# RishWijewardhena/vision-textile-inspection

Measured on AMD Instinct MI355X. Metric: frames/sec whole-node, YOLOv8n-seg 640x640 bs=64; mask IoU vs CPU ref, higher is better.
Workload: dtype f16x2

## Files before the change

include/vti.h:

```cpp
#ifndef VTI_H
#define VTI_H

#include <stddef.h>
#include <stdint.h>

#ifdef __cplusplus
extern "C" {
#endif

typedef struct vti_ctx vti_ctx;

typedef enum {
    VTI_OK = 0,
    VTI_ERR_ARG = -1,
    VTI_ERR_STATE = -2,
    VTI_ERR_WEIGHTS = -3,
    VTI_ERR_HIP = -4,
    VTI_ERR_NOMEM = -5,
    VTI_ERR_UNSUPPORTED = -6
} vti_status;

enum { VTI_F16 = 0, VTI_F32 = 1, VTI_H2 = 2 };
enum { VTI_MASK_LOGIT = 0,
       VTI_MASK_SIGMOID = 1 };
// ... 323 lines not shown
    const int32_t* classes;
} vti_nms_params;
VTI_NMS_TABLE_API int64_t vti_nms_table_bytes(int32_t n_rows);
VTI_NMS_TABLE_API int32_t vti_pack_nms_table(vti_ctx* ctx, const vti_nms_params* params, int32_t n_rows,
                                             void* host_table, size_t nbytes);
VTI_NMS_TABLE_API int32_t vti_set_nms_table(vti_ctx* ctx, const void* host_table, const void* dev_table,
                                            int32_t n_rows, const int32_t* dev_row_of_frame);

#define VTI_WINDOWS_API
VTI_WINDOWS_API int64_t vti_window_table_bytes(int32_t B);
VTI_WINDOWS_API int32_t vti_pack_windows(vti_ctx* ctx, int32_t H, int32_t W, const int32_t* H0, const int32_t* W0,
                                         const int64_t* byte_offset, const int32_t* windows, int32_t B, int64_t total_bytes,
                                         void* host_table, size_t nbytes);
VTI_WINDOWS_API int32_t vti_window_table_info(const void* host_table, int32_t b, int32_t out_i32[12], double out_f64[5]);
VTI_WINDOWS_API int32_t vti_letterbox_windows(vti_ctx* ctx, const uint8_t* dev_frames, const void* host_table, const void* dev_table,
                                              int32_t B, uint8_t* dev_input, void* stream);
VTI_WINDOWS_API int32_t vti_scale_boxes_windows(vti_ctx* ctx, const float* dev_dets, const int32_t* dev_counts, const void* host_table,
                                                const void* dev_table, int32_t B, int32_t max_det, float* dev_xyxy, void* stream);
VTI_WINDOWS_API int64_t vti_mask_native_windows_bytes(const vti_ctx* ctx, const void* host_table, int32_t max_det);
VTI_WINDOWS_API int32_t vti_masks_native_windows(vti_ctx* ctx, const float* dev_dets, const int32_t* dev_counts, const void* dev_proto,
                                                 const void* host_table, const void* dev_table, int32_t B, int32_t max_det, int32_t mode,
                                                 int32_t packing, uint8_t* dev_masks, int64_t capacity_bytes, int32_t* dev_offsets,
                                                 int64_t* dev_mask_bases, void* stream);
VTI_WINDOWS_API int32_t vti_predict_windows(vti_ctx* ctx, const uint8_t* dev_frames, const void* host_table, const void* dev_table,
                                            int32_t B, int32_t swap_rb, float conf, double iou, int32_t max_det, int32_t agnostic,
                                            int32_t mask_mode, int32_t packing, uint8_t* dev_input_scratch, float* dev_pred,
                                            void* dev_proto, float* dev_dets, int32_t* dev_counts, uint8_t* dev_masks,
                                            int64_t capacity_bytes, int32_t* dev_offsets, int64_t* dev_mask_bases, float* dev_xyxy,
                                            void* stream);

#define VTI_ANNOTATE_NATIVE_API
VTI_ANNOTATE_NATIVE_API int32_t vti_annotate_frames_native(vti_ctx* ctx, const uint8_t* dev_frames, const void* host_table,
                                                           const void* dev_table, int32_t B, const void* dev_cameras, int32_t n_cams,
                                                           const int32_t* dev_camera_of_frame, const uint8_t* dev_masks,
                                                           const int64_t* dev_mask_bases, int64_t capacity_bytes, const float* dev_dets,
                                                           const float* dev_xyxy, const int32_t* dev_counts, const int32_t* dev_offsets,
                                                           int32_t max_det, int32_t capacity, const int32_t* frame_i32,
                                                           const double* stitch_f64, const int32_t* stitch_i32,
                                                           const int32_t* host_select, const int32_t* dev_select, int32_t n_sel,
                                                           int32_t max_points, const void* host_out_table, const void* dev_out_table,
                                                           uint8_t* dev_out, int32_t* dev_status, void* dev_scratch, size_t scratch_bytes,
                                                           void* stream);
VTI_ANNOTATE_NATIVE_API int32_t vti_annotate_checker_frames_native(vti_ctx* ctx, const uint8_t* dev_frames, const void* host_table,
                                                                   const void* dev_table, int32_t B, const void* dev_cameras,
                                                                   int32_t n_cams, const int32_t* dev_camera_of_frame,
                                                                   const uint8_t* dev_masks, const int64_t* dev_mask_bases,
                                                                   int64_t capacity_bytes, const float* dev_dets, const float* dev_xyxy,
                                                                   const int32_t* dev_counts, const int32_t* dev_offsets, int32_t max_det,
                                                                   int32_t capacity, const int32_t* frame_i32, const double* stitch_f64,
                                                                   const int32_t* stitch_i32, const int32_t* host_select,
                                                                   const int32_t* dev_select, int32_t n_sel, int32_t max_points,
                                                                   const void* host_out_table, const void* dev_out_table,
                                                                   uint8_t* dev_out, int32_t* dev_status, void* dev_scratch,
                                                                   size_t scratch_bytes, void* stream);

int64_t vti_decode_jpeg_table_bytes(int32_t n);
int32_t vti_decode_jpeg_plan(vti_ctx* ctx, const uint8_t* host_files, const int64_t* host_file_offsets, int32_t n,
                             int32_t segment_bytes, int32_t layout, void* host_table, size_t nbytes, int32_t* out_H0,
                             int32_t* out_W0, int64_t* out_byte_offsets, int64_t* out_scratch_bytes);
enum { VTI_JPEG_CORRUPT = 1 };
int32_t vti_decode_jpeg(vti_ctx* ctx, const uint8_t* dev_files, const void* host_table, const void* dev_table, int32_t n, int32_t rgb,
                        uint8_t* dev_out, int64_t out_bytes, int32_t* dev_info, void* dev_scratch, size_t scratch_bytes, void* stream);

enum { VTI_RAW_YUYV = 0, VTI_RAW_UYVY, VTI_RAW_NV12, VTI_RAW_NV21, VTI_RAW_I420, VTI_RAW_YV12 };
int64_t vti_raw_frame_bytes(int32_t fmt, int32_t H0, int32_t W0);
int32_t vti_convert_raw(vti_ctx* ctx, const uint8_t* dev_raw, int32_t fmt, int32_t B, int32_t H0, int32_t W0, int32_t rgb,
                        uint8_t* dev_frames, void* stream);
int64_t vti_raw_table_bytes(int32_t n);
int32_t vti_pack_raw_frames(vti_ctx* ctx, const int32_t* H0, const int32_t* W0, const int32_t* fmt, int32_t n, void* host_raw_table,
                            size_t nbytes, int64_t* out_raw_offsets);
int32_t vti_convert_raw_frames(vti_ctx* ctx, const uint8_t* dev_raw, int64_t raw_bytes, const void* host_raw_table,
                               const void* dev_raw_table, const void* host_frame_table, const void* dev_frame_table, int32_t n,
                               int32_t rgb, uint8_t* dev_out, int64_t out_bytes, void* stream);

int32_t vti_debug_conv_output(vti_ctx* ctx, int32_t i, int32_t B, float* dev_out, void* stream);

int32_t vti_debug_conv2d(int32_t dtype, const void* dev_in, int32_t B, int32_t H, int32_t W, int32_t in_ld,
                         int32_t in_coff, int32_t c1, const float* host_w, const float* host_b, int32_t c2,
                         int32_t k, int32_t s, int32_t kind, const void* dev_res, int32_t res_ld, int32_t res_coff,
                         void* dev_out, int32_t out_ld, int32_t out_coff, int32_t out_f32, int32_t swap_rb,
                         int32_t tile_h, int32_t tile_w, int32_t waves_n, int32_t nrep, int32_t iters,
                         float* ms_out, int32_t* cfg_out, void* stream);

#ifdef __cplusplus
}
#endif
#endif
```

vision-textile-inspection_amd/_lib.py:

```python
import ctypes as C
import os

_HERE = os.path.dirname(os.path.abspath(__file__))
_VARIANT = os.environ.get("VTI_LIB_VARIANT", "")
LIB_PATH = os.path.join(_HERE, f"libvti_{_VARIANT}.so" if _VARIANT else "libvti.so")

VTI_F16, VTI_F32, VTI_H2 = 0, 1, 2
VTI_MASK_LOGIT, VTI_MASK_SIGMOID = 0, 1
VTI_PACK_U8, VTI_PACK_BITS = 0, 1
VTI_MASK_NATIVE = 0x10


class VtiDesc(C.Structure):
    _fields_ = [("scale", C.c_char), ("nc", C.c_int32), ("nm", C.c_int32), ("reg_max", C.c_int32),
                ("H", C.c_int32), ("W", C.c_int32), ("max_batch", C.c_int32), ("dtype", C.c_int32)]


class VtiConvInfo(C.Structure):
    _fields_ = [("name", C.c_char * 48), ("c1", C.c_int32), ("c2", C.c_int32), ("k", C.c_int32),
                ("s", C.c_int32), ("kind", C.c_int32), ("h_in", C.c_int32), ("w_in", C.c_int32),
                ("h_out", C.c_int32), ("w_out", C.c_int32), ("macs", C.c_int64),
                ("tile_h", C.c_int32), ("tile_w", C.c_int32), ("waves_n", C.c_int32), ("nrep", C.c_int32),
                ("lds_bytes", C.c_int32), ("fused", C.c_int32), ("persistent", C.c_int32)]

# ... 90 lines not shown
                                   _P, _P, _P, _P, _P]),
    "vti_frame_table_bytes": (_I64, [_I32]),
    "vti_pack_frames": (_I32, [_P, _I32, _I32, _P, _P, _P, _I32, _I64, _P, _SZ]),
    "vti_frame_table_info": (_I32, [_P, _I32, _P, _P]),
    "vti_letterbox_frames": (_I32, [_P, _P, _P, _P, _I32, _P, _P]),
    "vti_scale_boxes_frames": (_I32, [_P, _P, _P, _P, _P, _I32, _I32, _P, _P]),
    "vti_predict_frames": (_I32, [_P, _P, _P, _P, _I32, _I32, _F, _D, _I32, _I32, _I32, _I32,
                                  _P, _P, _P, _P, _P, _P, _I32, _P, _P, _P]),
    "vti_measure_frames": (_I32, [_P, _P, _I32, _P, _P, _I32, _P, _P, _P, _P, _P, _P, _I32, _I32, _I32, _P, _SZ,
                                  _P, _P, _P, _P, _P]),
    "vti_mask_native_frames_bytes": (_I64, [_P, _P, _I32]),
    "vti_masks_native_frames": (_I32, [_P, _P, _P, _P, _P, _P, _P, _I32, _I32, _I32, _I32, _P, _I64, _P, _P, _P]),
    "vti_predict_frames_native": (_I32, [_P, _P, _P, _P, _I32, _I32, _F, _D, _I32, _I32, _I32, _I32,
                                         _P, _P, _P, _P, _P, _P, _I64, _P, _P, _P, _P]),
    "vti_measure_frames_native": (_I32, [_P, _P, _I32, _P, _P, _P, _I64, _P, _P, _P, _P, _P, _P, _I32, _I32, _I32, _P, _SZ,
                                         _P, _P, _P, _P, _P]),
    "vti_mask_polygons_scratch_bytes": (_I64, [_P, _I32, _I32, _I32]),
    "vti_mask_polygons": (_I32, [_P, _P, _I32, _P, _I32, _I32, _I32, _I32, _I32, _I32, _P, _SZ, _P, _P, _I64, _P]),
    "vti_mask_polygons_frames_scratch_bytes": (_I64, [_P, _P, _I32]),
    "vti_mask_polygons_frames": (_I32, [_P, _P, _I32, _P, _I64, _P, _P, _P, _I32, _I32, _I32, _P, _SZ, _P, _P, _I64, _P]),
    "vti_annotate_scratch_bytes": (_I64, [_P, _I32, _I32, _I32, _I32, _I32]),
    "vti_annotate": (_I32, [_P, _P, _I32, _I32, _I32, _P, _I32, _P, _P, _I32, _P, _P, _P, _P, _I32, _I32, _P, _P, _P, _P, _P, _I32,
                            _I32, _P, _P, _P, _SZ, _P]),
    "vti_annotate_frames_scratch_bytes": (_I64, [_P, _P, _I32, _I32]),
    "vti_annotate_frames": (_I32, [_P, _P, _P, _P, _I32, _P, _I32, _P, _P, _I32, _P, _P, _P, _P, _I32, _I32, _P, _P, _P, _P, _P, _I32,
                                   _I32, _P, _P, _P, _P, _P, _SZ, _P]),
    "vti_annotate_checker": (_I32, [_P, _P, _I32, _I32, _I32, C.POINTER(VtiCheckerParams), _P, _I32, _P, _P, _P, _P, _I32, _I32, _P, _P, _P,
                                    _P, _P, _I32, _I32, _P, _P, _P, _SZ, _P]),
    "vti_checker_pack_cameras": (_I32, [_P, C.POINTER(VtiCheckerParams), _I32, _P, _SZ]),
    "vti_measure_checker_cameras": (_I32, [_P, _P, _I32, _P, _P, _I32, _P, _P, _P, _P, _I32, _I32, _I32, _I32, _I32, _P, _SZ,
                                           _P, _P, _P, _P, _P]),
    "vti_measure_checker_frames": (_I32, [_P, _P, _I32, _P, _P, _I32, _P, _P, _P, _P, _P, _P, _I32, _I32, _I32, _P, _SZ,
                                          _P, _P, _P, _P, _P]),
    "vti_measure_checker_frames_native": (_I32, [_P, _P, _I32, _P, _P, _P, _I64, _P, _P, _P, _P, _P, _P, _I32, _I32, _I32, _P, _SZ,
                                                 _P, _P, _P, _P, _P]),
    "vti_annotate_checker_cameras": (_I32, [_P, _P, _I32, _I32, _I32, _P, _I32, _P, _P, _I32, _P, _P, _P, _P, _I32, _I32, _P, _P, _P,
                                            _P, _P, _I32, _I32, _P, _P, _P, _SZ, _P]),
    "vti_annotate_checker_frames": (_I32, [_P, _P, _P, _P, _I32, _P, _I32, _P, _P, _I32, _P, _P, _P, _P, _I32, _I32, _P, _P, _P, _P, _P,
                                           _I32, _I32, _P, _P, _P, _P, _P, _SZ, _P]),
    "vti_annotate_frames_native": (_I32, [_P, _P, _P, _P, _I32, _P, _I32, _P, _P, _P, _I64, _P, _P, _P, _P, _I32, _I32, _P, _P, _P, _P, _P,
                                          _I32, _I32, _P, _P, _P, _P, _P, _SZ, _P]),
    "vti_annotate_checker_frames_native": (_I32, [_P, _P, _P, _P, _I32, _P, _I32, _P, _P, _P, _I64, _P, _P, _P, _P, _I32, _I32, _P, _P, _P,
                                                  _P, _P, _I32, _I32, _P, _P, _P, _P, _P, _SZ, _P]),
    "vti_overlay_scratch_bytes": (_I64, [_P, _I32, _I32, _I32, _I32, _I32]),
    "vti_overlay": (_I32, [_P, _P, _I32, _I32, _I32, _P, _I32, _P, _P, _P, _P, _I32, _I32, _P, _P, _I32, _F, _F, _P, _P, _I32, _I32, _P,
                           _I32, _P, _P, _P, _SZ, _P]),
    "vti_overlay_frames_scratch_bytes": (_I64, [_P, _P, _I32, _I32]),
    "vti_overlay_frames": (_I32, [_P, _P, _P, _P, _I32, _P, _I32, _P, _I64, _P, _P, _P, _P, _I32, _I32, _P, _P, _I32, _F, _F, _P, _P, _I32,
                                  _I32, _P, _I32, _P, _P, _P, _P, _P, _SZ, _P]),
    "vti_encode_jpeg_scratch_bytes": (_I64, [_P, _I32, _I32, _I32]),
    "vti_encode_jpeg_max_bytes": (_I64, [_I32, _I32, _I32]),
    "vti_encode_jpeg": (_I32, [_P, _P, _I32, _I32, _I32, _I32, _I32, _P, _SZ, _P, _P, _I64, _P]),
    "vti_encode_jpeg_frames_scratch_bytes": (_I64, [_P, _P]),
    "vti_encode_jpeg_frames_max_bytes": (_I64, [_P]),
    "vti_encode_jpeg_frames": (_I32, [_P, _P, _P, _P, _I32, _I32, _I32, _P, _SZ, _P, _P, _I64, _P]),
    "vti_stamp_table_bytes": (_I64, [_I32, _I32]),
    "vti_pack_stamps": (_I32, [_P, _P, _P, _I32, _P, _I32, _I64, _P, _SZ]),
    "vti_stamp": (_I32, [_P, _P, _I32, _I32, _I32, _P, _P, _P, _I64, _P]),
    "vti_stamp_frames": (_I32, [_P, _P, _P, _P, _I32, _P, _P, _P, _I64, _P]),
    "vti_nms_table_bytes": (_I64, [_I32]),
    "vti_pack_nms_table": (_I32, [_P, C.POINTER(VtiNmsParams), _I32, _P, _SZ]),
    "vti_set_nms_table": (_I32, [_P, _P, _P, _I32, _P]),
    "vti_window_table_bytes": (_I64, [_I32]),
    "vti_pack_windows": (_I32, [_P, _I32, _I32, _P, _P, _P, _P, _I32, _I64, _P, _SZ]),
    "vti_window_table_info": (_I32, [_P, _I32, _P, _P]),
    "vti_letterbox_windows": (_I32, [_P, _P, _P, _P, _I32, _P, _P]),
    "vti_scale_boxes_windows": (_I32, [_P, _P, _P, _P, _P, _I32, _I32, _P, _P]),
    "vti_mask_native_windows_bytes": (_I64, [_P, _P, _I32]),
    "vti_masks_native_windows": (_I32, [_P, _P, _P, _P, _P, _P, _I32, _I32, _I32, _I32, _P, _I64, _P, _P, _P]),
    "vti_predict_windows": (_I32, [_P, _P, _P, _P, _I32, _I32, _F, _D, _I32, _I32, _I32, _I32,
                                   _P, _P, _P, _P, _P, _P, _I64, _P, _P, _P, _P]),
    "vti_decode_jpeg_table_bytes": (_I64, [_I32]),
    "vti_decode_jpeg_plan": (_I32, [_P, _P, _P, _I32, _I32, _I32, _P, _SZ, _P, _P, _P, _P]),
    "vti_decode_jpeg": (_I32, [_P, _P, _P, _P, _I32, _I32, _P, _I64, _P, _P, _SZ, _P]),
    "vti_raw_frame_bytes": (_I64, [_I32, _I32, _I32]),
    "vti_convert_raw": (_I32, [_P, _P, _I32, _I32, _I32, _I32, _I32, _P, _P]),
    "vti_raw_table_bytes": (_I64, [_I32]),
    "vti_pack_raw_frames": (_I32, [_P, _P, _P, _P, _I32, _P, _SZ, _P]),
    "vti_convert_raw_frames": (_I32, [_P, _P, _I64, _P, _P, _P, _P, _I32, _I32, _P, _I64, _P]),
    "vti_debug_conv_output": (_I32, [_P, _I32, _I32, _P, _P]),
    "vti_debug_conv2d": (_I32, [_I32, _P, _I32, _I32, _I32, _I32, _I32, _I32, _P, _P, _I32, _I32, _I32, _I32,
                                _P, _I32, _I32, _P, _I32, _I32, _I32, _I32, _I32, _I32, _I32, _I32, _I32,
                                _P, _P, _P]),
}

_lib = None


def lib():
    global _lib
    if _lib is None:
        if not os.path.exists(LIB_PATH):
            raise ImportError(f"{LIB_PATH} not found: build it with `python -c 'import __graft_entry__ as g; "
                              f"g.build()'` (hipcc --offload-arch=gfx950); there is no CPU fallback")
        L = C.CDLL(LIB_PATH)
        for name, (res, args) in SIGNATURES.items():
            fn = getattr(L, name)
            fn.restype, fn.argtypes = res, args
        _lib = L
    return _lib


def check(ctx, rc):
    if rc != 0:
        msg = lib().vti_last_error(ctx)
        raise VtiError(rc, msg.decode() if msg else "")
```

vision-textile-inspection_amd/api.py:

```python
from ._lib import LIB_PATH, SIGNATURES, VtiError, lib
from .engine import Engine, FrameTable, WindowTable, NmsParams, NmsTable, RawTable, StampTable, debug_conv2d, h2_decode, h2_encode, kmeans1d2, pixels_to_world, unpack_bits
from .feeder import FrameFeeder
from .model import YOLO, Boxes, Masks, RawFrames, Results, letterbox_shape
from .weights import pack_container, random_weights, unpack_container
from .convert import convert_checkpoint, convert_state_dict
from .measure import CheckerParams, MeasureParams, MultiCameraChecker, MultiCameraMeasurer, StitchDistanceChecker, StitchMeasurer, checker_text_items
from .annotate import checker_display_list
from . import annotate, consumer, dataparallel, jpeg, overlay, rawframes

__all__ = ["LIB_PATH", "SIGNATURES", "VtiError", "lib", "Engine", "FrameTable", "WindowTable", "NmsParams", "NmsTable", "RawTable", "StampTable", "debug_conv2d", "h2_decode", "h2_encode", "kmeans1d2", "pixels_to_world", "unpack_bits", "FrameFeeder", "YOLO", "Boxes", "Masks", "RawFrames",
           "Results", "letterbox_shape", "pack_container", "random_weights", "unpack_container", "convert_checkpoint", "convert_state_dict",
           "MeasureParams", "MultiCameraMeasurer", "StitchMeasurer", "CheckerParams", "StitchDistanceChecker", "MultiCameraChecker", "checker_text_items", "checker_display_list", "annotate", "consumer", "dataparallel", "jpeg", "overlay", "rawframes"]
```

vision-textile-inspection_amd/csrc/misc.hip:

```cpp
#include "vti_internal.h"

namespace vti {

typedef _Float16 half_t;
typedef _Float16 half8 __attribute__((ext_vector_type(8)));
typedef float f32x4 __attribute__((ext_vector_type(4)));

typedef unsigned u32x4 __attribute__((ext_vector_type(4)));
struct h2e { unsigned u; };
__device__ __forceinline__ float h2_val(unsigned u) {
    return (float)__builtin_bit_cast(half_t, (unsigned short)(u & 0xffffu)) + (float)__builtin_bit_cast(half_t, (unsigned short)(u >> 16));
}

template <typename T> struct V16;
template <> struct V16<half_t> { typedef half8 vec; static constexpr int N = 8; };
template <> struct V16<float> { typedef f32x4 vec; static constexpr int N = 4; };
template <> struct V16<h2e> { typedef u32x4 vec; static constexpr int N = 4; };

__device__ __forceinline__ half8 vmax(half8 a, half8 b) { return __builtin_elementwise_max(a, b); }
__device__ __forceinline__ f32x4 vmax(f32x4 a, f32x4 b) { return __builtin_elementwise_max(a, b); }
__device__ __forceinline__ u32x4 vmax(u32x4 a, u32x4 b) {
    u32x4 r;
#pragma unroll
    for (int j = 0; j < 4; ++j) r[j] = h2_val(b[j]) > h2_val(a[j]) ? b[j] : a[j];
    return r;
}
template <typename T> __device__ __forceinline__ typename V16<T>::vec vlowest() {
    typename V16<T>::vec v;
    if constexpr (sizeof(T) == 4 && !__is_same(T, float)) {
#pragma unroll
        for (int j = 0; j < 4; ++j) v[j] = 0xfc00u;
    } else {
#pragma unroll
        for (int j = 0; j < V16<T>::N; ++j) v[j] = (T)(-INFINITY);
    }
    return v;
}

template <typename T>
__global__ __launch_bounds__(256) void sppf_pool_kernel(const PoolParams p) {
    using vec = typename V16<T>::vec;
    constexpr int N = V16<T>::N;
    const int cv = p.C / N;
    const long total = (long)p.B * p.H * p.W * cv;
    for (long i = blockIdx.x * 256L + threadIdx.x; i < total; i += (long)gridDim.x * 256) {
        const int c = (int)(i % cv);
        long r = i / cv;
        const int x = (int)(r % p.W); r /= p.W;
        const int y = (int)(r % p.H);
        const int b = (int)(r / p.H);
        const T* in = (const T*)p.in;
        vec m5 = vlowest<T>(), m9 = vlowest<T>(), m13 = vlowest<T>();
        for (int dy = -6; dy <= 6; ++dy) {
            const int yy = y + dy;
            if ((unsigned)yy >= (unsigned)p.H) continue;
            for (int dx = -6; dx <= 6; ++dx) {
                const int xx = x + dx;
                if ((unsigned)xx >= (unsigned)p.W) continue;
                const vec v = *(const vec*)(in + ((size_t)(b * p.H + yy) * p.W + xx) * p.ld + p.in_coff + c * N);
                const int ad = max(abs(dy), abs(dx));
                m13 = vmax(m13, v);
                if (ad <= 4) m9 = vmax(m9, v);
                if (ad <= 2) m5 = vmax(m5, v);
            }
        }
        T* o = (T*)p.out + ((size_t)(b * p.H + y) * p.W + x) * p.ld + p.out_coff + c * N;
        *(vec*)o = m5;
        *(vec*)(o + p.C) = m9;
        *(vec*)(o + 2 * p.C) = m13;
    }
}

template <typename T, int G>
__global__ __launch_bounds__(256) void sppf_pool_lds_kernel(const PoolParams p) {
    using vec = typename V16<T>::vec;
    constexpr int N = V16<T>::N;
    extern __shared__ __attribute__((aligned(16))) char smem[];
    const int HW = p.H * p.W;
    vec* cur = (vec*)smem;
    vec* tmp = cur + HW * G;
    const int cg = p.C / (N * G);
    const int b = blockIdx.x / cg, c = blockIdx.x - b * cg;
    const T* in = (const T*)p.in + (size_t)b * HW * p.ld + p.in_coff + c * (N * G);
    T* out = (T*)p.out + (size_t)b * HW * p.ld + p.out_coff + c * (N * G);
    {
        constexpr int MAXIT = 8;
        if (HW * G <= MAXIT * 256) {
            vec r[MAXIT];
#pragma unroll
            for (int it = 0; it < MAXIT; ++it) {
                const int i = threadIdx.x + it * 256;
                const int ic = i < HW * G ? i : 0;
                r[it] = *(const vec*)(in + (size_t)(ic / G) * p.ld + (ic % G) * N);
            }
#pragma unroll
            for (int it = 0; it < MAXIT; ++it) {
                const int i = threadIdx.x + it * 256;
                if (i < HW * G) cur[i] = r[it];
            }
        } else {
            for (int i = threadIdx.x; i < HW * G; i += 256) cur[i] = *(const vec*)(in + (size_t)(i / G) * p.ld + (i % G) * N);
        }
    }
    __syncthreads();
    for (int pass = 0; pass < 3; ++pass) {
        for (int i = threadIdx.x; i < HW * G; i += 256) {
            const int pix = i / G, v_ = i - pix * G;
            const int y = pix / p.W, x = pix - y * p.W;
            vec m = cur[i];
            for (int d = -2; d <= 2; ++d) {
                const int xx = x + d;
                if (d == 0 || (unsigned)xx >= (unsigned)p.W) continue;
                const vec v = cur[(y * p.W + xx) * G + v_];
                m = vmax(m, v);
            }
            tmp[i] = m;
        }
        __syncthreads();
        for (int i = threadIdx.x; i < HW * G; i += 256) {
            const int pix = i / G, v_ = i - pix * G;
            const int y = pix / p.W, x = pix - y * p.W;
            vec m = tmp[i];
            for (int d = -2; d <= 2; ++d) {
                const int yy = y + d;
                if (d == 0 || (unsigned)yy >= (unsigned)p.H) continue;
                const vec v = tmp[(yy * p.W + x) * G + v_];
                m = vmax(m, v);
            }
            cur[i] = m;
            *(vec*)(out + (size_t)pix * p.ld + pass * p.C + v_ * N) = m;
        }
        __syncthreads();
    }
}

hipError_t launch_sppf_pool(int dtype, const PoolParams& p, hipStream_t st) {
    const int N = dtype == VTI_F16 ? 8 : 4;
    const long total = (long)p.B * p.H * p.W * (p.C / N);
    if (total == 0) return hipSuccess;
    const size_t lds1 = (size_t)2 * p.H * p.W * 16;
    if (lds1 * 4 <= 64 * 1024 && p.C % (4 * N) == 0) {
        const int grid = p.B * (p.C / (4 * N));
        if (dtype == VTI_F16) hipLaunchKernelGGL((sppf_pool_lds_kernel<half_t, 4>), dim3(grid), dim3(256), lds1 * 4, st, p);
        else if (dtype == VTI_H2) hipLaunchKernelGGL((sppf_pool_lds_kernel<h2e, 4>), dim3(grid), dim3(256), lds1 * 4, st, p);
        else hipLaunchKernelGGL((sppf_pool_lds_kernel<float, 4>), dim3(grid), dim3(256), lds1 * 4, st, p);
        return hipGetLastError();
    }
    if (lds1 <= 64 * 1024) {
        const int grid = p.B * (p.C / N);
        if (dtype == VTI_F16) hipLaunchKernelGGL((sppf_pool_lds_kernel<half_t, 1>), dim3(grid), dim3(256), lds1, st, p);
        else if (dtype == VTI_H2) hipLaunchKernelGGL((sppf_pool_lds_kernel<h2e, 1>), dim3(grid), dim3(256), lds1, st, p);
        else hipLaunchKernelGGL((sppf_pool_lds_kernel<float, 1>), dim3(grid), dim3(256), lds1, st, p);
        return hipGetLastError();
    }
    const int grid = (int)((total + 255) / 256 < 4096 ? (total + 255) / 256 : 4096);
    if (dtype == VTI_F16) hipLaunchKernelGGL(sppf_pool_kernel<half_t>, dim3(grid), dim3(256), 0, st, p);
    else if (dtype == VTI_H2) hipLaunchKernelGGL(sppf_pool_kernel<h2e>, dim3(grid), dim3(256), 0, st, p);
    else hipLaunchKernelGGL(sppf_pool_kernel<float>, dim3(grid), dim3(256), 0, st, p);
    return hipGetLastError();
}

template <typename T>
__global__ __launch_bounds__(256) void upsample2x_kernel(const Up2Params p) {
    using vec = typename V16<T>::vec;
    constexpr int N = V16<T>::N;
    const int cv = p.C / N;
    const int Ho = 2 * p.H, Wo = 2 * p.W;
    const long total = (long)p.B * Ho * Wo * cv;
    for (long i = blockIdx.x * 256L + threadIdx.x; i < total; i += (long)gridDim.x * 256) {
        const int c = (int)(i % cv);
        long r = i / cv;
        const int x = (int)(r % Wo); r /= Wo;
        const int y = (int)(r % Ho);
        const int b = (int)(r / Ho);
        const vec v = *(const vec*)((const T*)p.in + ((size_t)(b * p.H + (y >> 1)) * p.W + (x >> 1)) * p.in_ld + p.in_coff + c * N);
        *(vec*)((T*)p.out + ((size_t)(b * Ho + y) * Wo + x) * p.out_ld + p.out_coff + c * N) = v;
    }
}

hipError_t launch_upsample2x(int dtype, const Up2Params& p, hipStream_t st) {
    const long total = (long)p.B * 4 * p.H * p.W * (p.C / (dtype == VTI_F16 ? 8 : 4));
    if (total == 0) return hipSuccess;
    const int grid = (int)((total + 255) / 256 < 4096 ? (total + 255) / 256 : 4096);
    if (dtype == VTI_F16) hipLaunchKernelGGL(upsample2x_kernel<half_t>, dim3(grid), dim3(256), 0, st, p);
    else hipLaunchKernelGGL(upsample2x_kernel<float>, dim3(grid), dim3(256), 0, st, p);
    return hipGetLastError();
}

constexpr int DEC_TA = 64;

__global__ __launch_bounds__(256) void decode_kernel(const DecodeParams p, int tiles0, int tiles1, int tiles_per_frame) {
    extern __shared__ __attribute__((aligned(16))) float tile[];
    const int b = blockIdx.x / tiles_per_frame;
    int t = blockIdx.x - b * tiles_per_frame;
    int l = 0;
    if (t >= tiles0 + tiles1) { l = 2; t -= tiles0 + tiles1; } else if (t >= tiles0) { l = 1; t -= tiles0; }
    const int W = p.W[l], HW = p.H[l] * W;
    const int la0 = t * DEC_TA;
    const int na = min(DEC_TA, HW - la0);
    const int nbox = 4 * p.reg_max, nin = nbox + p.nc + p.nm, pitch = nin + 1;
    const int tid = threadIdx.x;
    const size_t pix0 = (size_t)b * HW + la0;
    const float* src = p.box[l] + pix0 * nbox;
    for (int i = tid; i < na * nbox; i += 256) { const int a = i / nbox, k = i - a * nbox; tile[a * pitch + k] = src[i]; }
    src = p.cls[l] + pix0 * p.nc;
    for (int i = tid; i < na * p.nc; i += 256) { const int a = i / p.nc, k = i - a * p.nc; tile[a * pitch + nbox + k] = src[i]; }
    src = p.mc[l] + pix0 * p.nm;
    for (int i = tid; i < na * p.nm; i += 256) { const int a = i / p.nm, k = i - a * p.nm; tile[a * pitch + nbox + p.nc + k] = src[i]; }
    __syncthreads();
    float dist = 0.f;
    const int a_ = tid >> 2, side = tid & 3;
    if (a_ < na) {
        const float* v = tile + a_ * pitch + side * 16;
        float e[16];
        float mx = -INFINITY;
#pragma unroll
        for (int k = 0; k < 16; ++k) { e[k] = v[k]; mx = fmaxf(mx, e[k]); }
        float sum = 0.f;
#pragma unroll
        for (int k = 0; k < 16; ++k) { e[k] = expf(e[k] - mx); sum += e[k]; }
#pragma unroll
        for (int k = 0; k < 16; ++k) dist += (e[k] / sum) * (float)k;
    }
    __syncthreads();
    if (a_ < na) tile[a_ * pitch + side] = dist;
    __syncthreads();
    const int no = 4 + p.nc + p.nm;
    float* out = p.pred + ((size_t)b * p.A + p.a0[l] + la0) * no;
    const float st = (float)p.stride[l];
    for (int i = tid; i < no * DEC_TA; i += 256) {
        const int a = i / no, ch = i - a * no;
        if (a >= na) continue;
        const float* r = tile + a * pitch;
        float v;
        if (ch < 4) {
// ... 106 lines not shown
```

vision-textile-inspection_amd/csrc/vti_api.cpp:

```cpp
#include <algorithm>
#include <cmath>
#include <cstdio>
#include <cstdlib>
#include <cstring>
#include <new>

#include "vti_internal.h"
#include "rawframes_dev.h"

using namespace vti;

struct vti_ctx {
    Options opt;
    Plan plan;
    std::string err;
    int device = -1;
    void* d_wpk = nullptr;
    float* d_bias = nullptr;
    std::vector<float> alpha;
    char* ws = nullptr;
    size_t ws_bytes = 0;
    size_t act_bytes = 0;
    const void* last_input = nullptr;
    void* last_proto = nullptr;
// ... 2076 lines not shown
    }
    if (int32_t drc = check_device(c, "vti_convert_raw_frames")) return drc;
    VTI_HIP(c, launch_convert_raw_frames(raw_buf, dev_raw_table, frame_rows(dev_frame_table), n, max_items, rgb, out, (hipStream_t)stream),
            "convert_raw_frames kernel");
    return VTI_OK;
}

int32_t vti_debug_conv_output(vti_ctx* c, int32_t i, int32_t B, float* out, void* stream) {
    int32_t rc = check_ready(c, B, "vti_debug_conv_output");
    if (rc) return rc;
    if (i < 0 || i >= (int32_t)c->plan.convs.size() || !out) return fail(c, VTI_ERR_ARG, "vti_debug_conv_output: bad argument");
    const View& v = c->plan.conv_out[i];
    if (v.buf < 0) return fail(c, VTI_ERR_UNSUPPORTED, "vti_debug_conv_output: this conv is fused into the next one; its output is never materialised");
    const Buf& b = c->plan.bufs[v.buf];
    const void* src = buf_ptr(c->plan, bindings_of(c, c->last_input, nullptr, c->last_proto, nullptr), v.buf);
    if (!src) return fail(c, VTI_ERR_STATE, "vti_debug_conv_output: run vti_forward first");
    const int is_f32 = (b.elem == EL_F32 || (b.elem == EL_T && c->plan.desc.dtype == VTI_F32)) ? 1
                       : (b.elem == EL_T && c->plan.desc.dtype == VTI_H2) ? 2 : 0;
    VTI_HIP(c, launch_debug_nchw(is_f32, src, B, b.H, b.W, v.C, b.C, v.coff, out, (hipStream_t)stream), "debug copy");
    return VTI_OK;
}

int32_t vti_debug_conv2d(int32_t dtype, const void* dev_in, int32_t B, int32_t H, int32_t W, int32_t in_ld, int32_t in_coff,
                         int32_t c1, const float* host_w, const float* host_b, int32_t c2, int32_t k, int32_t s, int32_t kind,
                         const void* dev_res, int32_t res_ld, int32_t res_coff, void* dev_out, int32_t out_ld, int32_t out_coff,
                         int32_t out_f32, int32_t swap_rb, int32_t tile_h, int32_t tile_w, int32_t waves_n, int32_t nrep,
                         int32_t iters, float* ms_out, int32_t* cfg_out, void* stream) {
    if (!dev_in || !host_w || !host_b || !dev_out || B < 1 || H < 1 || W < 1 || c1 < 1 || c2 < 1 || iters < 1)
        return fail(nullptr, VTI_ERR_ARG, "vti_debug_conv2d: bad argument");
    if ((dtype != VTI_F16 && dtype != VTI_F32 && dtype != VTI_H2) || (kind < 0 || kind > 2))
        return fail(nullptr, VTI_ERR_ARG, "vti_debug_conv2d: bad dtype/kind");
    const bool conv0 = (c1 == 3);
    if (conv0 ? !(k == 3 && s == 2 && kind == 0) : (c1 % 16 != 0))
        return fail(nullptr, VTI_ERR_ARG, "vti_debug_conv2d: c1 must be 3 (stem) or a multiple of 16");
    if (!((k == 1 && s == 1) || (k == 3 && (s == 1 || s == 2)) || (kind == 2 && k == 2 && s == 2)))
        return fail(nullptr, VTI_ERR_ARG, "vti_debug_conv2d: unsupported kernel/stride");
    ConvRow r;
    r.name = "debug"; r.c1 = c1; r.c2 = c2; r.k = k; r.s = s; r.kind = kind; r.h_in = H; r.w_in = W;
    if (kind == 2) { r.h_out = 2 * H; r.w_out = 2 * W; }
    else { r.h_out = (H + 2 * (k / 2) - k) / s + 1; r.w_out = (W + 2 * (k / 2) - k) / s + 1; }
    const Options opt = options_from_env();
    ConvCfg g;
    choose_conv_cfg(opt.plan, dtype, r, conv0, B, g, tile_h, tile_w, waves_n, nrep);
    if (g.TH == 0) return fail(nullptr, VTI_ERR_ARG, "vti_debug_conv2d: no launch configuration fits");
    if (cfg_out) { cfg_out[0] = g.TH; cfg_out[1] = g.TW; cfg_out[2] = g.WN; cfg_out[3] = g.NREP; cfg_out[4] = (int32_t)g.lds * (g.pk ? -1 : 1); }
    std::vector<uint8_t> wpk(packed_conv_bytes(r, conv0, g));
    std::vector<float> bias((size_t)g.ntiles_n * 16);
    float alpha = 1.f;
    pack_conv(dtype, r, conv0, g, host_w, host_b, wpk.data(), bias.data(), 0, &alpha);
    void* d_w = nullptr; float* d_b = nullptr;
    hipStream_t st = (hipStream_t)stream;
    VTI_HIP(nullptr, hipMalloc(&d_w, wpk.size()), "hipMalloc");
    hipError_t e = hipMalloc((void**)&d_b, bias.size() * 4);
    if (e == hipSuccess) e = hipMemcpy(d_w, wpk.data(), wpk.size(), hipMemcpyHostToDevice);
    if (e == hipSuccess) e = hipMemcpy(d_b, bias.data(), bias.size() * 4, hipMemcpyHostToDevice);
    hipEvent_t e0 = nullptr, e1 = nullptr;
    if (e == hipSuccess) e = hipEventCreate(&e0);
    if (e == hipSuccess) e = hipEventCreate(&e1);
    if (e == hipSuccess) {
        LaunchRec L;
        conv_record(opt.run, dtype, r, g, B, dev_in, in_ld, in_coff, dev_out, out_ld, out_coff, dev_res, res_ld, res_coff, d_w, d_b, alpha,
                    out_f32 != 0, swap_rb, L);
#ifdef VTI_STAMPS
        (void)issue(L, st);
        (void)issue(L, st, "");
#endif
        e = issue(L, st);
        if (e == hipSuccess) e = hipEventRecord(e0, st);
        for (int i = 1; i < iters && e == hipSuccess; ++i) e = issue(L, st);
        if (e == hipSuccess) e = hipEventRecord(e1, st);
        if (e == hipSuccess) e = hipStreamSynchronize(st);
        float ms = 0.f;
        if (e == hipSuccess && iters > 1) e = hipEventElapsedTime(&ms, e0, e1);
        if (ms_out) *ms_out = iters > 1 ? ms / (iters - 1) : 0.f;
    }
    if (e0) (void)hipEventDestroy(e0);
    if (e1) (void)hipEventDestroy(e1);
    (void)hipFree(d_w);
    if (d_b) (void)hipFree(d_b);
    if (e != hipSuccess) return hip_fail(nullptr, e, "vti_debug_conv2d");
    return VTI_OK;
}

}
```

vision-textile-inspection_amd/engine.py:

```python
import contextlib
import ctypes as C
import dataclasses

import numpy as np
import torch

from . import _lib, rawframes
from . import overlay as _ov
from ._lib import VtiCheckerParams, VtiConvInfo, VtiDesc, VtiMeasureParams, VtiNmsParams, check, lib

DTYPES = {"fp16": _lib.VTI_F16, "f16": _lib.VTI_F16, "half": _lib.VTI_F16,
          "fp32": _lib.VTI_F32, "f32": _lib.VTI_F32, "float": _lib.VTI_F32,
          "h2": _lib.VTI_H2, "fp16x2": _lib.VTI_H2, "split": _lib.VTI_H2}
_DTYPE_NAME = {_lib.VTI_F16: "fp16", _lib.VTI_F32: "fp32", _lib.VTI_H2: "h2"}
MASK_MODES = {"logit": _lib.VTI_MASK_LOGIT, "sigmoid": _lib.VTI_MASK_SIGMOID}
PACKINGS = {"u8": _lib.VTI_PACK_U8, "bits": _lib.VTI_PACK_BITS}
POLY_STRATEGIES = {"largest": _lib.VTI_POLY_LARGEST, "concat": _lib.VTI_POLY_CONCAT}


def _ptr(t):
    return C.c_void_p(t.data_ptr()) if t is not None else C.c_void_p(0)


def _stream():
# ... 1291 lines not shown

def _f64(a, n):
    a = np.ascontiguousarray(np.asarray(a, dtype=np.float64).ravel())
    if a.size != n:
        raise ValueError(f"expected {n} float64 values, got {a.size}")
    return a


def pixels_to_world(uv, K, dist, R, t):
    uv = uv.to(torch.float64).contiguous()
    n = uv.shape[0]
    xyz = torch.empty((n, 3), dtype=torch.float64, device=uv.device)
    valid = torch.empty((n,), dtype=torch.int32, device=uv.device)
    Kh, dh, Rh, th = _f64(K, 9), _f64(dist, 5), _f64(R, 9), _f64(t, 3)
    rc = lib().vti_pixels_to_world(None, _ptr(uv), n, Kh.ctypes.data_as(C.c_void_p), dh.ctypes.data_as(C.c_void_p),
                                   Rh.ctypes.data_as(C.c_void_p), th.ctypes.data_as(C.c_void_p), _ptr(xyz), _ptr(valid), _stream())
    check(None, rc)
    return xyz, valid


def kmeans1d2(values, counts, max_iters=10):
    values = values.to(torch.float64).contiguous()
    B, max_n = values.shape
    labels = torch.empty((B, max_n), dtype=torch.int32, device=values.device)
    centers = torch.empty((B, 2), dtype=torch.float64, device=values.device)
    check(None, lib().vti_kmeans1d2(None, _ptr(values), _ptr(counts), B, max_n, int(max_iters), _ptr(labels), _ptr(centers), _stream()))
    return labels, centers


H2_SCALE = 16.0
H2_MAX = 4094.0


def h2_encode(t):
    s = t.float().clamp(-H2_MAX, H2_MAX) * H2_SCALE + 0.0
    hi = s.half()
    lo = (s - hi.float()).half()
    bits = hi.view(torch.int16).to(torch.int32) & 0xFFFF | (lo.view(torch.int16).to(torch.int32) << 16)
    return bits.view(torch.float32)


def h2_decode(t):
    bits = t.view(torch.int32)
    hi = (bits & 0xFFFF).to(torch.int16).view(torch.float16).float()
    lo = (bits >> 16).to(torch.int16).view(torch.float16).float()
    return (hi + lo) / H2_SCALE


def unpack_bits(bits, W):
    b = bits.unsqueeze(-1)
    sh = torch.arange(8, device=bits.device, dtype=torch.uint8)
    full = ((b >> sh) & 1).reshape(*bits.shape[:-1], bits.shape[-1] * 8)
    return full if full.shape[-1] == W else full[..., :W]


def to_numpy(t):
    return t.detach().cpu().numpy() if isinstance(t, torch.Tensor) else np.asarray(t)


def debug_conv2d(x, w, b, k, s, kind=0, dtype="fp16", res=None, out=None, in_coff=0, c1=None, out_coff=0, out_ld=None,
                 out_f32=False, swap_rb=False, tile=(0, 0), waves_n=0, nrep=0, iters=1):
    B, H, W, ld = x.shape
    w = np.ascontiguousarray(to_numpy(w), dtype=np.float32)
    b = np.ascontiguousarray(to_numpy(b), dtype=np.float32)
    c2 = w.shape[1] if kind == 2 else w.shape[0]
    if c1 is None:
        c1 = w.shape[0] if kind == 2 else w.shape[1]
    Ho, Wo = (2 * H, 2 * W) if kind == 2 else ((H + 2 * (k // 2) - k) // s + 1, (W + 2 * (k // 2) - k) // s + 1)
    tdt = torch.float32 if (out_f32 or DTYPES[dtype] != _lib.VTI_F16) else torch.float16
    if out is None:
        out_ld = out_ld or (out_coff + c2)
        out = torch.zeros((B, Ho, Wo, out_ld), dtype=tdt, device=x.device)
    else:
        out_ld = out.shape[3]
    ms = C.c_float(0)
    cfg = (C.c_int32 * 5)()
    rc = lib().vti_debug_conv2d(DTYPES[dtype], _ptr(x), B, H, W, ld, in_coff, c1, w.ctypes.data_as(C.c_void_p),
                                b.ctypes.data_as(C.c_void_p), c2, k, s, kind, _ptr(res), res.shape[3] if res is not None else 0,
                                0, _ptr(out), out_ld, out_coff, int(out_f32), int(swap_rb), tile[0], tile[1], waves_n, nrep,
                                iters, C.byref(ms), cfg, _stream())
    if rc != 0:
        raise _lib.VtiError(rc, lib().vti_last_error(None).decode())
    return out, ms.value, dict(tile=(cfg[0], cfg[1]), waves_n=cfg[2], nrep=cfg[3], lds=abs(cfg[4]), pk=cfg[4] < 0)
```

Measured before the change: 16220.

## Rewrite SPPF max-pool as sliding-window strip passes in LDS

Replaces the SPPF pooling kernel, which read five neighbours per element with a temp buffer, with an in-place strip kernel. Each thread slides a 5-wide window along a row or column strip of 32-bit words, keeping values in registers so each input is read once per pass. This halves LDS use since no tmp buffer is needed, and launches up to 512 threads per block. It adds a debug entry point for testing the pool alone. The SPPF layer is a small share of YOLOv8n, so the effect on whole-model throughput is likely small.

After: 16320 (median of 6 runs). About the same (+0.6%).

```diff
diff --git a/include/vti.h b/include/vti.h
--- a/include/vti.h
+++ b/include/vti.h
@@ -429,6 +429,10 @@
                          int32_t tile_h, int32_t tile_w, int32_t waves_n, int32_t nrep, int32_t iters,
                          float* ms_out, int32_t* cfg_out, void* stream);
 
+#define VTI_DEBUG_POOL_API
+VTI_DEBUG_POOL_API int32_t vti_debug_sppf_pool(int32_t dtype, const void* dev_in, int32_t B, int32_t H, int32_t W, int32_t C,
+                            int32_t ld, int32_t in_coff, int32_t out_coff, void* dev_out, void* stream);
+
 #ifdef __cplusplus
 }
 #endif
diff --git a/vision-textile-inspection_amd/_lib.py b/vision-textile-inspection_amd/_lib.py
--- a/vision-textile-inspection_amd/_lib.py
+++ b/vision-textile-inspection_amd/_lib.py
@@ -196,6 +196,7 @@
     "vti_debug_conv2d": (_I32, [_I32, _P, _I32, _I32, _I32, _I32, _I32, _I32, _P, _P, _I32, _I32, _I32, _I32,
                                 _P, _I32, _I32, _P, _I32, _I32, _I32, _I32, _I32, _I32, _I32, _I32, _I32,
                                 _P, _P, _P]),
+    "vti_debug_sppf_pool": (_I32, [_I32, _P, _I32, _I32, _I32, _I32, _I32, _I32, _I32, _P, _P]),
 }
 
 _lib = None
diff --git a/vision-textile-inspection_amd/api.py b/vision-textile-inspection_amd/api.py
--- a/vision-textile-inspection_amd/api.py
+++ b/vision-textile-inspection_amd/api.py
@@ -1,5 +1,5 @@
 from ._lib import LIB_PATH, SIGNATURES, VtiError, lib
-from .engine import Engine, FrameTable, WindowTable, NmsParams, NmsTable, RawTable, StampTable, debug_conv2d, h2_decode, h2_encode, kmeans1d2, pixels_to_world, unpack_bits
+from .engine import Engine, FrameTable, WindowTable, NmsParams, NmsTable, RawTable, StampTable, debug_conv2d, debug_sppf_pool, h2_decode, h2_encode, kmeans1d2, pixels_to_world, unpack_bits
 from .feeder import FrameFeeder
 from .model import YOLO, Boxes, Masks, RawFrames, Results, letterbox_shape
 from .weights import pack_container, random_weights, unpack_container
@@ -8,6 +8,6 @@
 from .annotate import checker_display_list
 from . import annotate, consumer, dataparallel, jpeg, overlay, rawframes
 
-__all__ = ["LIB_PATH", "SIGNATURES", "VtiError", "lib", "Engine", "FrameTable", "WindowTable", "NmsParams", "NmsTable", "RawTable", "StampTable", "debug_conv2d", "h2_decode", "h2_encode", "kmeans1d2", "pixels_to_world", "unpack_bits", "FrameFeeder", "YOLO", "Boxes", "Masks", "RawFrames",
+__all__ = ["LIB_PATH", "SIGNATURES", "VtiError", "lib", "Engine", "FrameTable", "WindowTable", "NmsParams", "NmsTable", "RawTable", "StampTable", "debug_conv2d", "debug_sppf_pool", "h2_decode", "h2_encode", "kmeans1d2", "pixels_to_world", "unpack_bits", "FrameFeeder", "YOLO", "Boxes", "Masks", "RawFrames",
            "Results", "letterbox_shape", "pack_container", "random_weights", "unpack_container", "convert_checkpoint", "convert_state_dict",
            "MeasureParams", "MultiCameraMeasurer", "StitchMeasurer", "CheckerParams", "StitchDistanceChecker", "MultiCameraChecker", "checker_text_items", "checker_display_list", "annotate", "consumer", "dataparallel", "jpeg", "overlay", "rawframes"]
diff --git a/vision-textile-inspection_amd/csrc/misc.hip b/vision-textile-inspection_amd/csrc/misc.hip
--- a/vision-textile-inspection_amd/csrc/misc.hip
+++ b/vision-textile-inspection_amd/csrc/misc.hip
@@ -71,86 +71,127 @@
     }
 }
 
+template <typename T> struct PoolLane;
+template <> struct PoolLane<h2e> {
+    static constexpr bool kDupNoop = true;
+    unsigned u; float f;
+    __device__ __forceinline__ void set(unsigned d) { u = d; f = h2_val(d); }
+    __device__ __forceinline__ void take(const PoolLane& b) { const bool g = b.f > f; u = g ? b.u : u; f = g ? b.f : f; }
+    __device__ __forceinline__ unsigned bits() const { return u; }
+};
+template <> struct PoolLane<half_t> {
+    static constexpr bool kDupNoop = false;
+    typedef _Float16 half2_t __attribute__((ext_vector_type(2)));
+    half2_t h;
+    __device__ __forceinline__ void set(unsigned d) { h = __builtin_bit_cast(half2_t, d); }
+    __device__ __forceinline__ void take(const PoolLane& b) { h = __builtin_elementwise_max(h, b.h); }
+    __device__ __forceinline__ unsigned bits() const { return __builtin_bit_cast(unsigned, h); }
+};
+template <> struct PoolLane<float> {
+    static constexpr bool kDupNoop = false;
+    float f;
+    __device__ __forceinline__ void set(unsigned d) { f = __builtin_bit_cast(float, d); }
+    __device__ __forceinline__ void take(const PoolLane& b) { f = __builtin_elementwise_max(f, b.f); }
+    __device__ __forceinline__ unsigned bits() const { return __builtin_bit_cast(unsigned, f); }
+};
+
+template <typename T, bool STORE>
+__device__ __forceinline__ void pool_strip(unsigned* l, const int st, const int n, unsigned* g, const size_t gst) {
+    unsigned raw[8];
+    PoolLane<T> w[8];
+    auto step = [&](const int x, const int k, const bool m2, const bool m1) {
+        raw[(k + 5) & 7] = l[min(x + 5, n - 1) * st];
+        w[(k + 2) & 7].set(raw[(k + 2) & 7]);
+        PoolLane<T> m = w[k];
+        if (m2) m.take(w[(k + 6) & 7]);
+        if (m1) m.take(w[(k + 7) & 7]);
+        if (PoolLane<T>::kDupNoop || x + 1 < n) m.take(w[(k + 1) & 7]);
+        if (PoolLane<T>::kDupNoop || x + 2 < n) m.take(w[(k + 2) & 7]);
+        l[x * st] = m.bits();
+        if constexpr (STORE) g[(size_t)x * gst] = m.bits();
+    };
+#pragma unroll
+    for (int q = 0; q < 5; ++q) raw[q] = l[min(q, n - 1) * st];
+    w[0].set(raw[0]);
+    w[1].set(raw[1]);
+    step(0, 0, false, false);
+    if (n > 1) step(1, 1, false, true);
+    for (int x0 = 2; x0 < n; x0 += 8) {
+#pragma unroll
+        for (int k = 0; k < 8; ++k) {
+            if (x0 + k >= n) break;
+            step(x0 + k, (k + 2) & 7, true, true);
+        }
+    }
+}
+
 template <typename T, int G>
-__global__ __launch_bounds__(256) void sppf_pool_lds_kernel(const PoolParams p) {
-    using vec = typename V16<T>::vec;
-    constexpr int N = V16<T>::N;
-    extern __shared__ __attribute__((aligned(16))) char smem[];
+__global__ __launch_bounds__(512) void sppf_pool_strip_kernel(const PoolParams p) {
+    extern __shared__ __attribute__((aligned(16))) unsigned smem_u[];
+    constexpr int DW = 4 / (int)sizeof(T) > 0 ? 4 / (int)sizeof(T) : 1;
     const int HW = p.H * p.W;
-    vec* cur = (vec*)smem;
-    vec* tmp = cur + HW * G;
-    const int cg = p.C / (N * G);
+    const int ldw = p.ld / DW, cw = p.C / DW;
+    const int cg = cw / G;
     const int b = blockIdx.x / cg, c = blockIdx.x - b * cg;
-    const T* in = (const T*)p.in + (size_t)b * HW * p.ld + p.in_coff + c * (N * G);
-    T* out = (T*)p.out + (size_t)b * HW * p.ld + p.out_coff + c * (N * G);
+    const unsigned* in = (const unsigned*)((const T*)p.in + (size_t)b * HW * p.ld + p.in_coff) + c * G;
+    unsigned* out = (unsigned*)((T*)p.out + (size_t)b * HW * p.ld + p.out_coff) + c * G;
+    const int nt = blockDim.x;
     {
-        constexpr int MAXIT = 8;
-        if (HW * G <= MAXIT * 256) {
-            vec r[MAXIT];
+        constexpr int MAXIT = 8, GV = G / 4;
+        const int nv = HW * GV;
+        if (nv <= MAXIT * nt) {
+            u32x4 r[MAXIT];
 #pragma unroll
             for (int it = 0; it < MAXIT; ++it) {
-                const int i = threadIdx.x + it * 256;
-                const int ic = i < HW * G ? i : 0;
-                r[it] = *(const vec*)(in + (size_t)(ic / G) * p.ld + (ic % G) * N);
+                const int i = threadIdx.x + it * nt;
+                const int ic = i < nv ? i : 0;
+                r[it] = *(const u32x4*)(in + (size_t)(ic / GV) * ldw + (ic % GV) * 4);
             }
 #pragma unroll
             for (int it = 0; it < MAXIT; ++it) {
-                const int i = threadIdx.x + it * 256;
-                if (i < HW * G) cur[i] = r[it];
+                const int i = threadIdx.x + it * nt;
+                if (i < nv) *(u32x4*)(smem_u + i * 4) = r[it];
             }
         } else {
-            for (int i = threadIdx.x; i < HW * G; i += 256) cur[i] = *(const vec*)(in + (size_t)(i / G) * p.ld + (i % G) * N);
-        }
-    }
-    __syncthreads();
-    for (int pass = 0; pass < 3; ++pass) {
-        for (int i = threadIdx.x; i < HW * G; i += 256) {
-            const int pix = i / G, v_ = i - pix * G;
-            const int y = pix / p.W, x = pix - y * p.W;
-            vec m = cur[i];
-            for (int d = -2; d <= 2; ++d) {
-                const int xx = x + d;
-                if (d == 0 || (unsigned)xx >= (unsigned)p.W) continue;
-                const vec v = cur[(y * p.W + xx) * G + v_];
-                m = vmax(m, v);
-            }
-            tmp[i] = m;
+            for (int i = threadIdx.x; i < nv; i += nt) *(u32x4*)(smem_u + i * 4) = *(const u32x4*)(in + (size_t)(i / GV) * ldw + (i % GV) * 4);
+        }
+    }
+    __syncthreads();
+    for (int level = 0; level < 3; ++level) {
+        for (int s0 = 0; s0 < p.H * G; s0 += nt) {
+            const int s = s0 + threadIdx.x;
+            if (s < p.H * G) pool_strip<T, false>(smem_u + (s / G) * (p.W * G) + s % G, G, p.W, nullptr, 0);
         }
         __syncthreads();
-        for (int i = threadIdx.x; i < HW * G; i += 256) {
-            const int pix = i / G, v_ = i - pix * G;
-            const int y = pix / p.W, x = pix - y * p.W;
-            vec m = tmp[i];
-            for (int d = -2; d <= 2; ++d) {
-                const int yy = y + d;
-                if (d == 0 || (unsigned)yy >= (unsigned)p.H) continue;
-                const vec v = tmp[(yy * p.W + x) * G + v_];
-                m = vmax(m, v);
-            }
-            cur[i] = m;
-            *(vec*)(out + (size_t)pix * p.ld + pass * p.C + v_ * N) = m;
-        }
-        __syncthreads();
-    }
+        for (int s0 = 0; s0 < p.W * G; s0 += nt) {
+            const int s = s0 + threadIdx.x;
+            if (s < p.W * G) pool_strip<T, true>(smem_u + s, p.W * G, p.H, out + (size_t)(s / G) * ldw + level * cw + s % G, (size_t)p.W * ldw);
+        }
+        if (level < 2) __syncthreads();
+    }
+}
+
+template <int G>
+static void launch_pool_strip(int dtype, const PoolParams& p, int grid, hipStream_t st) {
+    const int strips = (p.H > p.W ? p.H : p.W) * G;
+    const int nt = strips >= 512 ? 512 : (strips + 63) / 64 * 64;
+    const size_t lds = (size_t)p.H * p.W * G * 4;
+    if (dtype == VTI_F16) hipLaunchKernelGGL((sppf_pool_strip_kernel<half_t, G>), dim3(grid), dim3(nt), lds, st, p);
+    else if (dtype == VTI_H2) hipLaunchKernelGGL((sppf_pool_strip_kernel<h2e, G>), dim3(grid), dim3(nt), lds, st, p);
+    else hipLaunchKernelGGL((sppf_pool_strip_kernel<float, G>), dim3(grid), dim3(nt), lds, st, p);
 }
 
 hipError_t launch_sppf_pool(int dtype, const PoolParams& p, hipStream_t st) {
     const int N = dtype == VTI_F16 ? 8 : 4;
     const long total = (long)p.B * p.H * p.W * (p.C / N);
     if (total == 0) return hipSuccess;
-    const size_t lds1 = (size_t)2 * p.H * p.W * 16;
-    if (lds1 * 4 <= 64 * 1024 && p.C % (4 * N) == 0) {
-        const int grid = p.B * (p.C / (4 * N));
-        if (dtype == VTI_F16) hipLaunchKernelGGL((sppf_pool_lds_kernel<half_t, 4>), dim3(grid), dim3(256), lds1 * 4, st, p);
-        else if (dtype == VTI_H2) hipLaunchKernelGGL((sppf_pool_lds_kernel<h2e, 4>), dim3(grid), dim3(256), lds1 * 4, st, p);
-        else hipLaunchKernelGGL((sppf_pool_lds_kernel<float, 4>), dim3(grid), dim3(256), lds1 * 4, st, p);
+    const size_t lds4 = (size_t)p.H * p.W * 16;
+    if (lds4 * 4 <= 64 * 1024 && p.C % (4 * N) == 0) {
+        launch_pool_strip<16>(dtype, p, p.B * (p.C / (4 * N)), st);
         return hipGetLastError();
     }
-    if (lds1 <= 64 * 1024) {
-        const int grid = p.B * (p.C / N);
-        if (dtype == VTI_F16) hipLaunchKernelGGL((sppf_pool_lds_kernel<half_t, 1>), dim3(grid), dim3(256), lds1, st, p);
-        else if (dtype == VTI_H2) hipLaunchKernelGGL((sppf_pool_lds_kernel<h2e, 1>), dim3(grid), dim3(256), lds1, st, p);
-        else hipLaunchKernelGGL((sppf_pool_lds_kernel<float, 1>), dim3(grid), dim3(256), lds1, st, p);
+    if (lds4 <= 64 * 1024) {
+        launch_pool_strip<4>(dtype, p, p.B * (p.C / N), st);
         return hipGetLastError();
     }
     const int grid = (int)((total + 255) / 256 < 4096 ? (total + 255) / 256 : 4096);
diff --git a/vision-textile-inspection_amd/csrc/vti_api.cpp b/vision-textile-inspection_amd/csrc/vti_api.cpp
--- a/vision-textile-inspection_amd/csrc/vti_api.cpp
+++ b/vision-textile-inspection_amd/csrc/vti_api.cpp
@@ -2182,4 +2182,18 @@
     return VTI_OK;
 }
 
-}
+int32_t vti_debug_sppf_pool(int32_t dtype, const void* dev_in, int32_t B, int32_t H, int32_t W, int32_t C, int32_t ld, int32_t in_coff,
+                            int32_t out_coff, void* dev_out, void* stream) {
+    if (!dev_in || !dev_out || B < 1 || H < 1 || W < 1 || C < 1 || in_coff < 0 || out_coff < 0)
+        return fail(nullptr, VTI_ERR_ARG, "vti_debug_sppf_pool: bad argument");
+    if (dtype != VTI_F16 && dtype != VTI_F32 && dtype != VTI_H2) return fail(nullptr, VTI_ERR_ARG, "vti_debug_sppf_pool: bad dtype");
+    const int n = dtype == VTI_F16 ? 8 : 4;
+    if (C % n || ld % n || in_coff % n || out_coff % n || in_coff + C > ld || out_coff + 3 * C > ld)
+        return fail(nullptr, VTI_ERR_ARG, "vti_debug_sppf_pool: C, ld and the offsets must be multiples of 16 bytes, the slices inside ld");
+    PoolParams p;
+    p.in = dev_in; p.out = dev_out; p.B = B; p.H = H; p.W = W; p.C = C; p.ld = ld; p.in_coff = in_coff; p.out_coff = out_coff;
+    VTI_HIP(nullptr, launch_sppf_pool(dtype, p, (hipStream_t)stream), "vti_debug_sppf_pool");
+    return VTI_OK;
+}
+
+}
diff --git a/vision-textile-inspection_amd/engine.py b/vision-textile-inspection_amd/engine.py
--- a/vision-textile-inspection_amd/engine.py
+++ b/vision-textile-inspection_amd/engine.py
@@ -1397,3 +1397,12 @@
     if rc != 0:
         raise _lib.VtiError(rc, lib().vti_last_error(None).decode())
     return out, ms.value, dict(tile=(cfg[0], cfg[1]), waves_n=cfg[2], nrep=cfg[3], lds=abs(cfg[4]), pk=cfg[4] < 0)
+
+
+def debug_sppf_pool(x, C, in_coff, out_coff, dtype="fp16", out=None):
+    B, H, W, ld = x.shape
+    out = x if out is None else out
+    rc = lib().vti_debug_sppf_pool(DTYPES[dtype], _ptr(x), B, H, W, C, ld, in_coff, out_coff, _ptr(out), _stream())
+    if rc != 0:
+        raise _lib.VtiError(rc, lib().vti_last_error(None).decode())
+    return out
```
